# alipay/MMLRec-A-Unified-Multi-Task-and-Multi-Scenario-Learning-Benchmark-for-Recommendation

Hardware: AMD Instinct MI355X
Metric: train-step samples/sec, MMoE AliExpress-shape batch (higher is better)
Workload: dtype f32 (GEMMs: fp32-equivalent emulation on the 16-bit MFMA pipe with f32 accumulate -- two scaled fp16 planes per operand where the operand magnitudes travel with the tensors (batches >= 32 768), else three bf16 planes; max-norm error vs float64 3.3e-7 / 4.7e-7, fp32 MFMA 4.3e-7); 1 GPU; mmoe_ae30: 30 sparse fields, 12.49M rows (1e+07-row top table), E=8, mmoe 4 experts, experts [256, 128], gates [64], towers [64], adam lr 0.005; batch_per_gpu=65536, global_batch=65536, index_dist=zipf, table_update=dense_exact, dense_update_schedule=one launch after the scatter, gradients read for marked rows only, hip_graph=True, scatter_mode=deterministic, streams=1, early_fork=0, tables=single GPU

## Files before the change

### include/mmlrec.h

```cpp
#ifndef MMLREC_H
#define MMLREC_H

#include <stdint.h>

#ifdef __cplusplus
extern "C" {
#endif

#define MML_OK 0
#define MML_ERR_ARG (-1)
#define MML_ERR_HIP (-2)
#define MML_ERR_UNSUPPORTED (-3)

#define MML_MAX_FIELDS 64
#define MML_MAX_GROUP 16
#define MML_MAX_SRC 8
#define MML_MAX_EXPERTS 16
#define MML_MAX_GATES 8
#define MML_MAX_HEADS 8
#define MML_MAX_OPT_TENSORS 32
#define MML_AMAX_WORDS 8
#define MML_MAX_AMAX 64

typedef void* mml_stream_t;
// ... 525 lines not shown
  float* dV[2];
  float* dK[2];
  float* dQ[2];
  int64_t lddv[2], lddk[2], lddq[2];
  int64_t B;
  int32_t H;
  float sqrt_h;
} mml_attn2_desc;
int mml_attn2_fwd(const mml_attn2_desc* d, mml_stream_t stream);
int mml_attn2_bwd(const mml_attn2_desc* d, mml_stream_t stream);
int mml_esmm_combine(const float* p_raw, int64_t ldr, const float* y, int64_t ldy, const float* d_out, int64_t lddo,
                     float* p_out, int64_t ldo, float* d_raw, int64_t lddr, float* loss, int64_t B, mml_stream_t stream);
int mml_apg_features_fwd(const float* o1, int64_t ldo1, const float* s, int64_t lds, float* z, int64_t ldz, int64_t B,
                         int32_t k, int32_t E, int32_t Kf, mml_stream_t stream);
int mml_apg_features_bwd(const float* dz, int64_t lddz, const float* s, int64_t lds, float* do1, int64_t lddo1,
                         int64_t B, int32_t k, int32_t E, int32_t accumulate, mml_stream_t stream);
int mml_apg_weights(float* Wkk, float* bkk, float* Wb, float* Wcat, int64_t ldw, int32_t k, int32_t E, int32_t dir,
                    int32_t acc_kk, int32_t acc_bkk, int32_t acc_wb, mml_stream_t stream);
int mml_escm_combine(const float* p_raw, int64_t ldr, const float* y, int64_t ldy, const float* d_out, int64_t lddo,
                     float* p_out, int64_t ldo, float* d_raw, int64_t lddr, float* loss, int64_t B, float cf_w,
                     float global_w, mml_stream_t stream);
int mml_auc_segments(const float* pred, int64_t ldp, const float* y, int64_t ldy, int64_t n, int32_t cols, int32_t seg,
                     double* auc, mml_stream_t stream);
int32_t mml_auc_sorted_tile(void);
int64_t mml_auc_sorted_workspace_bytes(int64_t n, int32_t cols, int64_t seg);
int mml_auc_sorted(const float* pred, int64_t ldp, const float* y, int64_t ldy, const float* mask, int64_t ldm,
                   int32_t mask_cols, int64_t n, int32_t cols, int64_t seg, void* workspace, int64_t workspace_bytes,
                   double* auc, int64_t* counts, int32_t* status, mml_stream_t stream);
int mml_act_bwd(const float* y, const float* dy, float* dst, int64_t n, int32_t act, mml_stream_t stream);

typedef struct {
  float* param; const float* grad;
  float* state1;
  float* state2;
  int64_t n;
  float l1, l2;
  const uint32_t* skip_rows;
  int32_t row_elems;
  int32_t zero_grads;
  uint8_t* grad_marks;
  int64_t* acc64;
  const uint32_t* acc_amax;
  int32_t acc_shift;
  int32_t acc_pad_;
  uint8_t* warm_rows;
} mml_opt_tensor;
typedef struct {
  int32_t kind;
  int32_t step;
  const int32_t* step_dev;
  float lr, beta1, beta2, eps, alpha;
  int32_t zero_grad;
  int32_t max_blocks;
} mml_opt_hyper;
int mml_opt_step_dense(const mml_opt_tensor* tensors, int32_t n, const mml_opt_hyper* hyper, mml_stream_t stream);
int mml_opt_step_rows(float* const* tables, float* const* grad_tables, float* const* state1, float* const* state2,
                      uint32_t* const* seen, const int64_t* rowbase, int32_t F, int32_t E,
                      const int32_t* touched, const int32_t* touched_count, int32_t touched_cap,
                      int32_t* const* last ,
                      const mml_opt_hyper* hyper, mml_stream_t stream);
int mml_opt_catchup_rows(float* const* tables, float* const* state1, float* const* state2, int32_t* const* last,
                         const int64_t* rowbase, int32_t F, int32_t E, const int32_t* touched,
                         const int32_t* touched_count, int32_t touched_cap, const mml_opt_hyper* hyper,
                         mml_stream_t stream);
int mml_opt_catchup_dense(float* table, float* state1, float* state2, int32_t* last, int64_t V, int32_t E,
                          const mml_opt_hyper* hyper, mml_stream_t stream);
int mml_counter_update(int32_t* counter, int32_t delta, int32_t reset, mml_stream_t stream);

#ifdef __cplusplus
}
#endif
#endif
```

### mmlrec-a-unified-multi-task-and-multi-scenario-learning-benchmark-for-recommendation_amd/_lib.py

```python
import ctypes as C
import os

import torch

from . import build as _build

MAX_FIELDS, MAX_GROUP, MAX_SRC, MAX_EXPERTS, MAX_GATES, MAX_HEADS, MAX_OPT_TENSORS = 64, 16, 8, 16, 8, 8, 32
OPT_STREAM_MIN_PARAMS, OPT_HUGE_MIN_PARAMS, OPT_STREAM_MAX_TENSORS = 1 << 24, 1 << 22, 4
MAX_POOLED, POOL_MAX_LEN = 16, 256
POOL_COMBINERS = {"sum": 0, "mean": 1, "max": 2}
ACT_NONE, ACT_RELU, ACT_SIGMOID, ACT_SIGMOID2 = 0, 1, 2, 3
HEAD_OUT_SIGMOID, HEAD_OUT_IDENTITY = 0, 1
HEAD_LOSS_BCE, HEAD_LOSS_MSE, HEAD_LOSS_MAE = 0, 1, 2


def head_kind(out=HEAD_OUT_SIGMOID, loss=HEAD_LOSS_BCE):
    return (int(loss) << 8) | int(out)


ERR_ARG = -1
SCATTER_DET_CLEAR_MARKS, SCATTER_DET_AMAX_SUPPLIED, SCATTER_DET_DEFER_TOTALS = 1, 2, 4
OPT_SGD, OPT_ADAM, OPT_ADAGRAD, OPT_RMSPROP = 0, 1, 2, 3
OPT_KINDS = {"sgd": OPT_SGD, "adam": OPT_ADAM, "adagrad": OPT_ADAGRAD, "rmsprop": OPT_RMSPROP}

# ... 105 lines not shown
                ("amax_dH", fp), ("amax_dA", fp), ("K", i32), ("N", i32), ("n_hbias2", i32), ("mask_col", i32),
                ("head", i32), ("kind", i32)]


class TowerHeadGroup(C.Structure):
    _fields_ = [("n", i32), ("pad_", i32), ("M", i64), ("prob", fp), ("ldprob", i64), ("y", fp), ("ldy", i64),
                ("mask", fp), ("ldmask", i64), ("loss", fp), ("t", TowerHeadDesc * MAX_HEADS)]


class OptTensor(C.Structure):
    _fields_ = [("param", fp), ("grad", fp), ("state1", fp), ("state2", fp), ("n", i64), ("l1", C.c_float),
                ("l2", C.c_float), ("skip_rows", fp), ("row_elems", i32), ("zero_grads", i32), ("grad_marks", fp),
                ("acc64", fp), ("acc_amax", fp), ("acc_shift", i32), ("acc_pad_", i32), ("warm_rows", fp)]


class Copy2dDesc(C.Structure):
    _fields_ = [("src", fp), ("lds", i64), ("dst", fp), ("ldd", i64), ("rows", i64), ("cols", i32),
                ("accumulate", i32), ("amax_out", fp)]


class PreluDesc(C.Structure):
    _fields_ = [("z", fp), ("ldz", i64), ("y", fp), ("ldy", i64), ("rows", i64), ("cols", i32), ("pad_", i32),
                ("alpha", fp), ("amax_out", fp)]


class PreluBwdDesc(C.Structure):
    _fields_ = [("dy", fp), ("lddy", i64), ("z", fp), ("ldz", i64), ("dz", fp), ("lddz", i64), ("rows", i64),
                ("cols", i32), ("pad_", i32), ("alpha", fp), ("dalpha", fp), ("accumulate_dz", i32),
                ("accumulate_dalpha", i32), ("amax_out", fp)]


PCGRAD_MAX_TASKS = 8


class PcgradSeg(C.Structure):
    _fields_ = [("bank", fp * PCGRAD_MAX_TASKS), ("out", fp), ("rows", i64), ("ld", i64), ("cols", i32), ("pad_", i32),
                ("row_marks", fp)]


class SumProdDesc(C.Structure):
    _fields_ = [("out", fp), ("x", fp * 8), ("y", fp * 8), ("n", i64), ("n_terms", i32), ("accumulate", i32),
                ("deriv_of", fp), ("act", i32), ("pad_", i32), ("amax_out", fp)]


class Attn2Desc(C.Structure):
    _fields_ = [("V", fp * 2), ("K", fp * 2), ("Q", fp * 2), ("ldv", i64 * 2), ("ldk", i64 * 2), ("ldq", i64 * 2),
                ("out", fp), ("ldo", i64), ("A", fp), ("dout", fp), ("lddo", i64), ("dV", fp * 2), ("dK", fp * 2),
                ("dQ", fp * 2), ("lddv", i64 * 2), ("lddk", i64 * 2), ("lddq", i64 * 2), ("B", i64), ("H", i32),
                ("sqrt_h", C.c_float)]


class OptHyper(C.Structure):
    _fields_ = [("kind", i32), ("step", i32), ("step_dev", fp), ("lr", C.c_float), ("beta1", C.c_float),
                ("beta2", C.c_float), ("eps", C.c_float), ("alpha", C.c_float), ("zero_grad", i32), ("max_blocks", i32)]


_PP = C.POINTER
_SIGS = {
    "mml_version": (C.c_int, []),
    "mml_last_error": (C.c_char_p, []),
    "mml_device_caps": (C.c_int, [C.c_int, _PP(i64)]),
    "mml_stream_create_cu_range": (C.c_int, [C.c_int, C.c_int, C.c_int, _PP(C.c_void_p)]),
    "mml_stream_destroy": (C.c_int, [C.c_void_p]),
    "mml_gather_fwd": (C.c_int, [_PP(fp), _PP(i64), _PP(i32), i32, i32, fp, i64, i32, i32, i64, fp, i64, fp, fp]),
    "mml_gather_wgmax_len": (i64, [i32, i32, i32, i64]),
    "mml_gather_fwd_wgmax": (C.c_int, [_PP(fp), _PP(i64), _PP(i32), i32, i32, fp, i64, i32, i32, i64, fp, i64, fp, i64, fp, fp]),
    "mml_gather_fwd_mark": (C.c_int, [_PP(fp), _PP(i64), _PP(i32), i32, i32, fp, i64, i32, i32, i64, fp, i64, fp, fp, fp]),
    "mml_rows_compact": (C.c_int, [_PP(fp), _PP(i64), _PP(i64), i32, fp, fp, i32, fp, fp]),
    "mml_gather_fwd_idx32": (C.c_int, [_PP(fp), _PP(i64), i32, i32, fp, i64, fp, i64, i32, i64, fp, i64, fp, fp]),
    "mml_scatter_bwd": (C.c_int, [_PP(fp), _PP(i64), _PP(i32), i32, i32, fp, i64, i64, fp, i64, _PP(fp), _PP(i64),
                                  fp, fp, i32, fp, fp, fp]),
    "mml_scatter_bwd_det": (C.c_int, [_PP(fp), _PP(i64), _PP(i32), i32, i32, fp, i64, i64, fp, i64, _PP(fp), fp, fp, i32,
                                      fp, fp]),
    "mml_scatter_det_shift": (i32, [i64]),
    "mml_scatter_bwd_idx32": (C.c_int, [_PP(fp), _PP(i64), i32, i32, fp, i64, i64, fp, i64, _PP(fp), _PP(i64),
                                        fp, fp, i32, fp, fp, fp]),
    "mml_index_unique_idx32": (C.c_int, [_PP(i64), i32, i32, fp, i64, i64, _PP(fp), _PP(i64), fp, fp, i32, fp, fp, fp]),
    "mml_route_count": (C.c_int, [fp, i64, fp, i64, _PP(i32), _PP(i64), i32, i64, i32, fp, fp, fp]),
    "mml_route_place": (C.c_int, [fp, i64, fp, i64, _PP(i32), _PP(i64), _PP(i64), i32, i64, i32, fp, fp, fp, fp, fp]),
    "mml_rows_permute": (C.c_int, [fp, i64, fp, i32, i32, i64, fp, fp]),
    "mml_route_list_count": (C.c_int, [fp, fp, i32, _PP(i64), _PP(i64), i32, i32, fp, fp]),
    "mml_route_list_place": (C.c_int, [fp, fp, i32, _PP(i64), _PP(i64), _PP(i64), i32, i32, fp, fp, fp, fp]),
    "mml_lookup_slots": (C.c_int, [fp, i64, _PP(i32), _PP(i64), _PP(i64), i32, i64, fp, fp, fp, fp]),
    "mml_rows_clear": (C.c_int, [fp, fp, i32, _PP(i64), _PP(fp), i32, fp]),
    "mml_shard_rows": (C.c_int, [fp, i64, fp, i64, i32, i32, i32, i32, fp]),
    "mml_amax_batch": (C.c_int, [_PP(AmaxDesc), i32, fp]),
    "mml_amax_reset": (C.c_int, [fp, i64, fp]),
    "mml_gemm_planes_cut": (C.c_int, [C.POINTER(PlanesDesc), i32, fp]),
    "mml_gemm_set_mode": (C.c_int, [i32]),
    "mml_gemm_get_mode": (C.c_int, []),
    "mml_gemm_set_panel": (C.c_int, [i32]),
    "mml_gemm_set_ws": (C.c_int, [i32]),
    "mml_gemm_set_nt": (C.c_int, [i32]),
    "mml_gemm_nt_serves": (C.c_int, [_PP(GemmWgradDesc)]),
    "mml_gemm_os_serves": (C.c_int, [_PP(GemmDgradDesc), i32]),
    "mml_tower_head_serves": (C.c_int, [_PP(TowerHeadGroup)]),
    "mml_tower_head_workspace_bytes": (i64, [_PP(TowerHeadGroup)]),
    "mml_tower_head_fwd_bwd": (C.c_int, [_PP(TowerHeadGroup), fp, i64, i32, fp]),
    "mml_gemm_last_kernel": (C.c_char_p, []),
    "mml_gather_last_kernel": (C.c_char_p, []),
    "mml_gemm_set_wgrad_lds_pad": (C.c_int, [i32]),
    "mml_cast16_batch": (C.c_int, [_PP(Cast16Desc), i32, fp]),
    "mml_gather16_fwd": (C.c_int, [_PP(fp), _PP(i64), _PP(i32), i32, i32, fp, i64, i32, i32, i64, fp, i64, fp, fp]),
    "mml_g16_tn": (C.c_int, [_PP(G16TnDesc), i32, fp]),
    "mml_g16_wgrad_workspace_bytes": (i64, [_PP(G16WgradDesc), i32]),
    "mml_g16_wgrad": (C.c_int, [_PP(G16WgradDesc), i32, fp, i64, i32, fp]),
    "mml_g16_last_kernel": (C.c_char_p, []),
# ... 122 lines not shown
```

### mmlrec-a-unified-multi-task-and-multi-scenario-learning-benchmark-for-recommendation_amd/csrc/optim_ew.hip

```cpp
#include "common.hpp"
#include "fold_fixed.hpp"

#include <stdlib.h>

#ifndef MML_OPT_COLD_CB
#define MML_OPT_COLD_CB 8
#endif

namespace mml {

struct OptLaunch {
  mml_opt_tensor t[MML_MAX_OPT_TENSORS];
  int32_t n;
  int32_t variant;
  mml_opt_hyper h;
  int64_t chunk0[MML_MAX_OPT_TENSORS + 1];
  int32_t blk0[MML_MAX_OPT_TENSORS + 1];
  int32_t prop;
};
static_assert(sizeof(OptLaunch) <= 4096, "OptLaunch travels by value: the kernel-argument block holds 4 KB");

struct StepConsts {
  float step_size;
  float inv_bc2s;
// ... 117 lines not shown
      if (t0.x | t0.y) A64[2 * c] = lzero;
      if (t1.x | t1.y) A64[2 * c + 1] = lzero;
    };
    int64_t i = tid;
    if (PATH == OPT_UNROLL2 && !skip && !gm) {
      for (; i + stride < n4; i += 2 * stride) {
        const int64_t j = i + stride;
        f4 p0 = ld(P + i), p1 = ld(P + j);
        const f4 g0 = ld(G + i), g1 = ld(G + j);
        f4 a0 = S1 ? ld(S1 + i) : zero, a1 = S1 ? ld(S1 + j) : zero;
        f4 b0 = S2 ? ld(S2 + i) : zero, b1 = S2 ? ld(S2 + j) : zero;
        one(p0, g0, a0, b0);
        one(p1, g1, a1, b1);
        st(P + i, p0);
        st(P + j, p1);
        if (S1) { st(S1 + i, a0); st(S1 + j, a1); }
        if (S2) { st(S2 + i, b0); st(S2 + j, b1); }
        if (h.zero_grad && (g0.x != 0.f || g0.y != 0.f || g0.z != 0.f || g0.w != 0.f)) G[i] = zero;
        if (h.zero_grad && (g1.x != 0.f || g1.y != 0.f || g1.z != 0.f || g1.w != 0.f)) G[j] = zero;
      }
    }
    if (PATH == OPT_SKIP_U && skip) {
      for (; i + (U - 1) * stride < n4; i += U * stride) {
        f4 p[U], a[U], b[U];
        uint32_t w[U];
#pragma unroll
        for (int k = 0; k < U; ++k) {
          const int64_t row = row_of(i + k * stride);
          w[k] = (skip[row >> 5] >> (row & 31)) & 1u;
        }
#pragma unroll
        for (int k = 0; k < U; ++k) {
          const int64_t j = i + k * stride;
          if (!w[k]) {
            p[k] = ld(P + j);
            a[k] = S1 ? ld(S1 + j) : zero;
            b[k] = S2 ? ld(S2 + j) : zero;
          }
        }
#pragma unroll
        for (int k = 0; k < U; ++k) {
          if (w[k]) continue;
          const int64_t j = i + k * stride;
          const f4 g = zg ? zero : ld(G + j);
          one(p[k], g, a[k], b[k]);
          st(P + j, p[k]);
          if (S1) st(S1 + j, a[k]);
          if (S2) st(S2 + j, b[k]);
          if (h.zero_grad && (g.x != 0.f || g.y != 0.f || g.z != 0.f || g.w != 0.f)) G[j] = zero;
        }
      }
    }
    uint8_t* const wr = gm ? T.warm_rows : nullptr;
    if ((PATH == OPT_MARK_U || PATH == OPT_MARK_ACC_U) && wr && !skip) {
      constexpr int CB = MML_OPT_COLD_CB;
      for (; i < n4; i += CB * stride) {
        uint32_t lm = 0, wm = 0;
#pragma unroll
        for (int k = 0; k < CB; ++k) {
          const int64_t j = i + k * stride;
          const bool in = j < n4;
          const int64_t row = row_of(in ? j : i);
          const uint8_t mk = gm[row], wk = wr[row];
          lm |= (uint32_t)(in && mk != 0) << k;
          wm |= (uint32_t)(in && wk != 0) << k;
        }
        const uint32_t act = lm | wm;
        if (__builtin_amdgcn_ballot_w64(act != 0) == 0) continue;
#pragma unroll 1
        for (int kk = 0; kk < CB; kk += 2) {
          if (__builtin_amdgcn_ballot_w64(((act >> kk) & 3u) != 0) == 0) continue;
          f4 p[2], a[2], b[2], g[2];
          l2 t0[2], t1[2];
#pragma unroll
          for (int k = 0; k < 2; ++k) {
            const int64_t j = i + (kk + k) * stride;
            const bool on = (act >> (kk + k)) & 1u, lv = (lm >> (kk + k)) & 1u;
            p[k] = a[k] = b[k] = g[k] = zero;
            t0[k] = t1[k] = lzero;
            if (on) {
              p[k] = ld(P + j);
              if (S1) a[k] = ld(S1 + j);
              if (S2) b[k] = ld(S2 + j);
            }
            if (lv) {
              if (!zg) g[k] = ld(G + j);
              if (PATH == OPT_MARK_ACC_U && A64) {
                t0[k] = A64[2 * j];
                t1[k] = A64[2 * j + 1];
              }
            }
          }
#pragma unroll
          for (int k = 0; k < 2; ++k) {
            const int64_t j = i + (kk + k) * stride;
            const bool on = (act >> (kk + k)) & 1u, lv = (lm >> (kk + k)) & 1u;
            if (!on) continue;
            f4 gs = g[k];
            if (PATH == OPT_MARK_ACC_U && A64 && lv) add_totals(gs, t0[k], t1[k], j);
            one(p[k], gs, a[k], b[k]);
            st(P + j, p[k]);
            if (S1) st(S1 + j, a[k]);
            if (S2) st(S2 + j, b[k]);
            if (h.zero_grad && (g[k].x != 0.f || g[k].y != 0.f || g[k].z != 0.f || g[k].w != 0.f)) G[j] = zero;
            const int64_t row = row_of(j);
            if (lv && (j << 2) == row * re) {
              gm[row] = 0;
// ... 618 lines not shown
}

extern "C" int mml_opt_step_dense(const mml_opt_tensor* tensors, int32_t n, const mml_opt_hyper* hyper,
                                  mml_stream_t stream) {
  int rc = check_hyper(hyper, "mml_opt_step_dense");
  if (rc) return rc;
  MML_REQUIRE(n >= 0 && (n == 0 || tensors), "mml_opt_step_dense: bad tensor array");
  int i = 0;
  while (i < n) {
    OptLaunch L{};
    L.h = *hyper;
    int64_t total = 0, chunks = 0;
    while (i < n && L.n < MML_MAX_OPT_TENSORS) {
      const mml_opt_tensor& t = tensors[i];
      MML_REQUIRE(t.param && t.grad && t.n >= 0, "mml_opt_step_dense: tensor %d malformed", i);
      MML_REQUIRE(hyper->kind == MML_OPT_SGD || t.state1, "mml_opt_step_dense: tensor %d needs state1", i);
      MML_REQUIRE(hyper->kind != MML_OPT_ADAM || t.state2, "mml_opt_step_dense: tensor %d needs state2 (Adam)", i);
      MML_REQUIRE(!t.skip_rows || (t.row_elems > 0 && t.row_elems % 4 == 0 && t.n % t.row_elems == 0 &&
                                   aligned16(t.param)),
                  "mml_opt_step_dense: tensor %d: skip_rows needs row_elems %% 4 == 0 dividing n and a 16-byte aligned "
                  "parameter (16-byte chunks must lie inside one row)", i);
      if (t.acc64) {
        MML_REQUIRE(t.grad_marks && !t.skip_rows && t.acc_amax && aligned16(t.acc64) && t.acc_shift >= 4 &&
                        t.acc_shift <= 28,
                    "mml_opt_step_dense: tensor %d: acc64 (deferred totals of mml_scatter_bwd_det) needs grad_marks, no "
                    "skip_rows, a 16-byte aligned int64 array, acc_amax and acc_shift = mml_scatter_det_shift(B)", i);
      }
      if (t.grad_marks) {
        const int cpr = t.row_elems / 4;
        MML_REQUIRE(t.row_elems > 0 && t.row_elems % 4 == 0 && cpr <= 64 && (cpr & (cpr - 1)) == 0 &&
                        t.n % t.row_elems == 0 && !t.skip_rows && aligned16(t.param) && aligned16(t.grad) &&
                        (!t.state1 || aligned16(t.state1)) && (!t.state2 || aligned16(t.state2)),
                    "mml_opt_step_dense: tensor %d: grad_marks needs 16-byte aligned [rows, row_elems] tensors with "
                    "row_elems / 4 a power of two <= 64 and no skip_rows", i);
      }
      if (t.warm_rows) {
        MML_REQUIRE(t.grad_marks && t.l1 == 0.f && t.l2 == 0.f,
                    "mml_opt_step_dense: tensor %d: warm_rows needs grad_marks and no regulariser (a regulariser moves a "
                    "row whose moments and gradient are zero)", i);
      }
      L.chunk0[L.n] = chunks;
      L.t[L.n++] = t;
      total += t.n;
      chunks += cdiv(t.n, 4);
      ++i;
    }
    L.chunk0[L.n] = chunks;
    if (total == 0) continue;
    static int variant = -1;
    if (variant < 0) {
      const char* e = getenv("MMLREC_OPT_VARIANT");
      variant = e ? atoi(e) : 0;
    }
    L.variant = variant | (hyper->max_blocks > 0 ? 4 : 0);
    int64_t nmax = 0;
    for (int k = 0; k < L.n; ++k) nmax = L.t[k].n > nmax ? L.t[k].n : nmax;
    bool all_gm = true, all_skip = true, none = true, any_acc = false;
    for (int k = 0; k < L.n; ++k) {
      any_acc = any_acc || L.t[k].acc64;
      all_gm = all_gm && L.t[k].grad_marks && !L.t[k].skip_rows;
      all_skip = all_skip && L.t[k].skip_rows;
      none = none && !L.t[k].grad_marks && !L.t[k].skip_rows;
    }
    const bool many = L.n > 4 && all_gm;
    MML_REQUIRE(!any_acc || all_gm, "mml_opt_step_dense: a launch with acc64 tensors takes grad_marks on every tensor");
    if (total >= ((int64_t)1 << 24) && (L.n <= 4 || many)) {
      int64_t bx = cdiv(cdiv(nmax, 4), 256);
      if (bx > 256 * 8) bx = 256 * 8;
      if (hyper->max_blocks > 0 && bx * L.n > hyper->max_blocks) bx = cdiv(hyper->max_blocks, L.n);
      dim3 grid((unsigned)bx, (unsigned)L.n);
      bool all_warm = true;
      for (int k = 0; k < L.n; ++k) all_warm = all_warm && L.t[k].warm_rows;
      static int cold_wgs = -1;
      if (cold_wgs < 0) {
        const char* e = getenv("MMLREC_OPT_COLD_WGS");
        cold_wgs = e ? atoi(e) : 256 * 8;
        if (cold_wgs < 1 || cold_wgs > 256 * 8) cold_wgs = 256 * 8;
      }
      const int64_t wg_cap = all_warm ? cold_wgs : 256 * 8;
      if (many) {
        int64_t want = 0;
        for (int k = 0; k < L.n; ++k) {
          const int64_t need = cdiv(cdiv(L.t[k].n, 4), 256);
          want += need > wg_cap ? wg_cap : (need < 1 ? 1 : need);
        }
        const bool capped = hyper->max_blocks > 0 && want > hyper->max_blocks;
        int64_t tb = capped ? hyper->max_blocks : want;
        if (tb < L.n) tb = L.n;
        int64_t at = 0;
        for (int k = 0; k < L.n; ++k) {
          L.blk0[k] = (int32_t)at;
          const int64_t need = cdiv(cdiv(L.t[k].n, 4), 256);
          int64_t nb = capped ? tb * L.t[k].n / total : (need > wg_cap ? wg_cap : need);
          if (nb > need) nb = need;
          if (nb < 1) nb = 1;
          at += nb;
        }
        L.blk0[L.n] = (int32_t)at;
        L.prop = 1;
        grid = dim3((unsigned)at, 1);
      }
      static int u_mark = -1;
      if (u_mark < 0) {
        const char* e = getenv("MMLREC_OPT_U");
        u_mark = e ? atoi(e) : 2;
      }
      hipStream_t st = to_stream(stream);
// ... 250 lines not shown
```

### mmlrec-a-unified-multi-task-and-multi-scenario-learning-benchmark-for-recommendation_amd/ops.py

```python
import ctypes as C

import os

import torch

from . import _lib as L

_workspaces = {}


def _stream():
    return torch.cuda.current_stream().cuda_stream


_masked_streams = {}


def cu_range_stream(device, cu_lo, cu_hi):
    idx = device.index if device.index is not None else torch.cuda.current_device()
    key = (idx, int(cu_lo), int(cu_hi))
    st = _masked_streams.get(key)
    if st is None:
        h = C.c_void_p()
        L.check(L.load().mml_stream_create_cu_range(idx, int(cu_lo), int(cu_hi), C.byref(h)))
# ... 779 lines not shown
                    (b.shape[-1] > 1 and b.stride(-1) != 1)):
                raise L.MMLError("pcgrad: banks and out of a segment must be float32 views of one shape and pitch")
        rows, cols = (1, ref.shape[0]) if ref.dim() == 1 else ref.shape
        for k, b in enumerate(banks):
            d.bank[k] = b.data_ptr() if b is not None else None
        d.out = L.ptr(sg.get("out"))
        d.rows, d.cols, d.ld = rows, cols, (cols if ref.dim() == 1 else _ld(ref))
        marks = sg.get("marks")
        if marks is not None and (marks.dtype != torch.uint8 or marks.numel() < rows or not marks.is_contiguous()):
            raise L.MMLError("pcgrad: marks must be a contiguous uint8 tensor with one byte per row")
        d.row_marks = L.ptr(marks)
        if need_out and sg.get("out") is None:
            raise L.MMLError("pcgrad combine: a segment without `out`")
    return arr


def pcgrad_gram(segs, T, gram=None):
    arr = make_pcgrad_segs(segs, T)
    dev = next(b for b in segs[0]["banks"] if b is not None).device
    if gram is None:
        gram = torch.empty((T, T), dtype=torch.float64, device=dev)
    nbytes = int(L.load().mml_pcgrad_workspace_bytes(arr, len(segs), T))
    ws = workspace(nbytes, dev)
    L.check(L.load().mml_pcgrad_gram(arr, len(segs), T, gram.data_ptr(), ws.data_ptr(), nbytes, _stream()),
            "mml_pcgrad_gram")
    return gram


def pcgrad_weights(gram, order, w=None, fired=None):
    _need_gpu(gram, order)
    T = gram.shape[0]
    if gram.dtype != torch.float64 or order.dtype != torch.int32 or order.numel() != T * T or gram.numel() != T * T \
            or not gram.is_contiguous() or not order.is_contiguous():
        raise L.MMLError("pcgrad_weights: gram [T, T] float64 and order [T, T] int32, contiguous")
    if w is None:
        w = torch.empty(2 * T, dtype=torch.float32, device=gram.device)
    if fired is None:
        fired = torch.empty((T, T), dtype=torch.int32, device=gram.device)
    L.check(L.load().mml_pcgrad_weights(gram.data_ptr(), order.data_ptr(), T, w.data_ptr(), fired.data_ptr(), _stream()),
            "mml_pcgrad_weights")
    return w, fired


def pcgrad_combine(segs, T, w):
    _need_gpu(w)
    arr = make_pcgrad_segs(segs, T, need_out=True)
    L.check(L.load().mml_pcgrad_combine(arr, len(segs), T, w.data_ptr(), _stream()), "mml_pcgrad_combine")


def act_bwd(y, dy, dst, act):
    L.check(L.load().mml_act_bwd(y.data_ptr(), dy.data_ptr(), dst.data_ptr(), y.numel(), act, _stream()), "mml_act_bwd")


def make_hyper(kind, lr, step=1, step_dev=None, zero_grad=False, max_blocks=0):
    h = L.OptHyper()
    h.kind = L.OPT_KINDS[kind] if isinstance(kind, str) else int(kind)
    h.step = int(step)
    h.step_dev = L.ptr(step_dev)
    h.lr = float(lr)
    h.beta1, h.beta2 = 0.9, 0.999
    h.eps = {L.OPT_ADAM: 1e-8, L.OPT_ADAGRAD: 1e-10, L.OPT_RMSPROP: 1e-8}.get(h.kind, 0.0)
    h.alpha = 0.99
    h.zero_grad = int(zero_grad)
    h.max_blocks = int(max_blocks)
    return h


def make_opt_tensors(entries):
    arr = (L.OptTensor * len(entries))()
    for d, ent in zip(arr, entries):
        p, g, s1, s2 = ent[:4]
        d.param, d.grad, d.state1, d.state2, d.n = p.data_ptr(), g.data_ptr(), L.ptr(s1), L.ptr(s2), p.numel()
        d.l1, d.l2 = ent[4] if len(ent) > 4 and ent[4] else (0.0, 0.0)
        if len(ent) > 5 and ent[5] is not None:
            d.skip_rows, d.row_elems, d.zero_grads = ent[5].data_ptr(), p.shape[1], 1
        if len(ent) > 6 and ent[6] is not None:
            d.grad_marks, d.row_elems = ent[6].data_ptr(), p.shape[1]
        if len(ent) > 7 and ent[7] is not None:
            d.acc64, d.acc_amax, d.acc_shift = ent[7][0].data_ptr(), ent[7][1].data_ptr(), int(ent[7][2])
        if len(ent) > 8 and ent[8] is not None:
            d.warm_rows = ent[8].data_ptr()
    return arr


def opt_step_dense(entries, hyper):
    arr = make_opt_tensors(entries)
    L.check(L.load().mml_opt_step_dense(arr, len(entries), C.byref(hyper), _stream()), "mml_opt_step_dense")


def opt_step_rows(tables, grad_tables, state1, state2, seen, rowbase, touched, touched_count, hyper, last=None):
    F, E = len(tables), tables[0].shape[1]
    rb = (L.i64 * (F + 1))(*rowbase)
    L.check(L.load().mml_opt_step_rows(_ptr_array(tables), _ptr_array(grad_tables),
                                       _ptr_array(state1) if state1 is not None else None,
                                       _ptr_array(state2) if state2 is not None else None,
                                       _ptr_array(seen), rb, F, E, touched.data_ptr(), touched_count.data_ptr(),
                                       touched.numel(), _ptr_array(last) if last is not None else None,
                                       C.byref(hyper), _stream()), "mml_opt_step_rows")


def index_unique(vocab, cols, E, X, seen, rowbase, touched, touched_count, status=None, marks=None):
    F = len(vocab)
    L.check(L.load().mml_index_unique((L.i64 * F)(*vocab), (L.i32 * F)(*cols), F, E, X.data_ptr(), _ld(X), X.shape[0],
                                      _ptr_array(seen), (L.i64 * (F + 1))(*rowbase), touched.data_ptr(),
                                      touched_count.data_ptr(), touched.numel(), L.ptr(marks), L.ptr(status), _stream()),
            "mml_index_unique")


# ... 188 lines not shown
```

### mmlrec-a-unified-multi-task-and-multi-scenario-learning-benchmark-for-recommendation_amd/optimizer.py

```python
import ctypes as C
import dataclasses
import os
import typing

import torch

from . import _lib as L
from . import engine as E
from . import ops


@dataclasses.dataclass(frozen=True)
class OptKnobs:
    lazy_min_params: int = 1 << 22
    auto_table_update: str = "lazy_exact"
    early_blocks: int = 0
    tail_blocks: int = 1 << 20
    opt_u: typing.Optional[int] = None
    one_launch: bool = False
    variant: int = 0
    scatter_old: bool = False
    cold_rows: bool = True

    @classmethod
    def from_env(cls, env=None):
        env = os.environ if env is None else env
        u = env.get("MMLREC_OPT_U")
        return cls(lazy_min_params=int(env.get("MMLREC_LAZY_MIN_PARAMS", str(1 << 22))),
                   auto_table_update=env.get("MMLREC_AUTO_TABLE_UPDATE", "lazy_exact"),
                   early_blocks=int(env.get("MMLREC_EARLY_BLOCKS", "0")),
                   tail_blocks=int(env.get("MMLREC_TAIL_BLOCKS", str(1 << 20))),
                   opt_u=int(u) if u is not None else None,
                   one_launch=env.get("MMLREC_OPT_ONE_LAUNCH", "0") == "1",
                   variant=int(env.get("MMLREC_OPT_VARIANT", "0")),
                   scatter_old=bool(env.get("MMLREC_SCATTER_OLD")),
                   cold_rows=env.get("MMLREC_OPT_COLD_ROWS", "1") != "0")


TABLE_UPDATES = ("dense_exact", "sparse_rows", "lazy_exact")
BYTES_PER_PARAM = {"sgd": 12, "adam": 28, "adagrad": 20, "rmsprop": 20}


def resolve_table_update(kind, requested, widths, one_table_per_field, table_params, table_reg, knobs):
    mode = requested
    if requested == "auto":
        if kind in ("sgd", "adagrad"):
            mode = "sparse_rows"
        else:
            ok = (len(widths) == 1 and widths <= {4, 8, 16} and one_table_per_field and
                  table_params > knobs.lazy_min_params and knobs.auto_table_update == "lazy_exact")
            mode = "lazy_exact" if ok else "dense_exact"
        if table_reg:
            mode = "dense_exact"
    if mode == "lazy_exact" and kind in ("sgd", "adagrad"):
        mode = "sparse_rows"
    if mode not in TABLE_UPDATES:
        raise ValueError("table_update must be auto, dense_exact, sparse_rows or lazy_exact")
    return mode


def opt_dense_symbol(numel, ntensors, form=0, opt_u=None):
    if not L.opt_dense_streams(numel, ntensors, form in (3, 4)):
        return "opt_flat_kernel"
    u = {0: 1, 1: 1, 2: 4, 3: 2 if opt_u is None else opt_u, 4: 4 if opt_u == 4 else 2}[form]
    return "opt_dense_kernel<true, %d, %d>" % (form, u)


class DenseLaunch(typing.NamedTuple):
    tables: tuple
    marked: bool
    form: int
    bytes: float
    kernel: str


def dense_table_launches(kind, numels, rows, marks, split_dense, cap, det_deferred, knobs, det_exact=True):
    n = len(numels)
    big = [i for i in range(n) if numels[i] >= L.OPT_HUGE_MIN_PARAMS]
    if len(big) > L.OPT_STREAM_MAX_TENSORS or sum(numels[i] for i in big) < L.OPT_STREAM_MIN_PARAMS:
        big = []
    small = [i for i in range(n) if i not in big]
    one_launch = bool(big and small and cap > 0 and n <= L.MAX_OPT_TENSORS and not split_dense and all(marks) and
                      knobs.one_launch)
    if det_deferred:
        if not (det_exact and L.opt_takes_det_totals(numels, all(marks), split_dense)):
            raise L.MMLError("the deterministic scatter deferred its totals to a marked dense update of exactly its "
                             "tables")
        one_launch = True
    if one_launch:
        big, small = small + big, []
    per = BYTES_PER_PARAM[kind] - (4 if split_dense else 0)
    out = []
    for grp in (big, small):
        if not grp:
            continue
        marked = grp is big and all(marks[i] for i in grp)
        numel = sum(numels[i] for i in grp)
        nbytes = float(per) * numel
        form = (4 if det_deferred else 3 if (cap > 0 and marked) else 2 if (cap > 0 and split_dense) else
                1 if (knobs.variant & 2 and not marked and not split_dense) else 0)
        if marked:
            nbytes += sum(rows[i] - 4.0 * numels[i] for i in grp)
        out.append(DenseLaunch(tuple(grp), marked, form, nbytes, opt_dense_symbol(numel, len(grp), form, knobs.opt_u)))
    return out


WARM_KINDS = ("adam", "rmsprop", "adagrad")


def launch_trusts_warm_map(kind, marked, table_reg, knobs, sharded=False):
    return bool(marked and kind in WARM_KINDS and not table_reg and knobs.cold_rows and not sharded)


class TableRows:

    def __init__(self, vocab, device, cap):
        self.rowbase = [0]
        for v in vocab:
            self.rowbase.append(self.rowbase[-1] + int(v))
        self.seen = [torch.zeros((int(v) + 31) // 32, dtype=torch.int32, device=device) for v in vocab]
        self.marks = torch.zeros(ops.marks_bytes(vocab), dtype=torch.uint8, device=device)
        self.touched = torch.zeros(max(int(cap), 1), dtype=torch.int32, device=device)
        self.count = torch.zeros(1, dtype=torch.int32, device=device)


class ParamStore:

    def __init__(self, model, device):
        self.device = device
        self.model = model
        tables, dense = [], []
        for name, p in model.named_parameters():
            (tables if name.startswith("embedding_dict.") else dense).append((name, p))
        self.sig = tuple(p.data_ptr() for _, p in tables + dense)
        total = sum(p.numel() for _, p in dense)
        self.arena = torch.zeros(max(total, 1), dtype=torch.float32, device=device)
        self.pvals = {}
        off = 0
        for name, p in dense:
            g = self.arena[off:off + p.numel()].view(p.shape)
            off += p.numel()
            self.pvals[name] = E.PVal(p.data, g, name)
            self.pvals[name].stable = True
        self.table_names = [n for n, _ in tables]
        for name, p in tables:
            self.pvals[name] = E.PVal(p.data, None, name, is_table=True)
        par = getattr(model, "_parallel", None)
        if par is not None and par.mode == "row_sharded":
            self.pvals["embedding_shard"] = E.PVal(par.shard, None, "embedding_shard", is_table=True)
            self.table_names = ["embedding_shard"]
        self.table_grads_ready = False
        self.opt = None
        self.rows = None
        self.rows_names = None
        self._grad_marks_key = self._det_key = None
        self.extra = {}

    def ensure_table_grads(self):
        if not self.table_grads_ready:
            for n in self.table_names:
                pv = self.pvals[n]
                pv.grad = torch.zeros_like(pv.data)
                pv.needs_grad = True
            self.table_grads_ready = True

    def ensure_rows(self, cap, names=None):
# ... 107 lines not shown
        return c["pre"] + c["early"] + c["mlp"] + c["tables"]

    def split_dense_ok(self, widths):
        return (self.table_update == "dense_exact" and not self.table_reg() and
                all(w <= 16 and w % 4 == 0 for w in widths))

    def can_split_dense(self, plan):
        gop = plan.ops[0] if plan.ops else None
        if not isinstance(gop, E.GatherOp) or isinstance(gop, E.PooledGatherOp):
            return False
        return self.split_dense_ok([t.data.shape[1] for t in gop.tables])

    def calls_split(self, plan, split_dense=False):
        knobs = OptKnobs.from_env()
        pre = [(L.load().mml_counter_update, (self.step_dev.data_ptr(), 1, 0))]
        if self.table_update == "lazy_exact":
            pre += self._lazy_pre_calls(plan)
        split_dense = bool(split_dense) and self.can_split_dense(plan)
        if split_dense and getattr(plan.ops[0], "mark_rows", None) is None:
            pre += self.index_pre_calls(plan)
        reg = self._reg_map()
        treg = self.table_reg(reg)
        names = [n for n in self.store.table_names if self.store.pvals[n].written]
        if treg and self.table_update != "dense_exact":
            raise NotImplementedError("l2_reg_embedding / l1 on the tables makes every row's gradient non-zero: use "
                                      "table_update='dense_exact' (the reference's own dense optimizer)")
        hyper = ops.make_hyper(self.kind, self.lr, step=0, step_dev=self.step_dev, zero_grad=False)
        plan.keep.append(hyper)
        mlp = self._mlp_calls(plan, reg, hyper)
        early, tables = [], []
        if names and self.table_update == "dense_exact":
            (early if split_dense else tables).extend(self._dense_table_calls(plan, names, treg, split_dense, knobs))
        if names and (self.table_update != "dense_exact" or split_dense):
            tables += self._row_update_calls(plan, names, hyper, knobs)
        return {"pre": pre, "early": early, "mlp": mlp, "tables": tables}

    def _mlp_calls(self, plan, reg, hyper):
        dense = [(pv, n) for n, pv in self.store.pvals.items()
                 if not pv.is_table and pv.grad is not None and (pv.written or pv.data.data_ptr() in reg)]
        if not dense:
            return []
        arr = ops.make_opt_tensors([(pv.data, pv.grad) + self.state[n] + (reg.get(pv.data.data_ptr()),)
                                    for pv, n in dense])
        plan.keep.append(arr)
        numel = sum(pv.data.numel() for pv, _ in dense)
        return [(L.load().mml_opt_step_dense, (arr, len(dense), C.byref(hyper)),
                 dict(kernel=opt_dense_symbol(numel, len(dense)), bytes=float(BYTES_PER_PARAM[self.kind]) * numel))]

    def _dense_table_calls(self, plan, names, treg, split_dense, knobs):
        st = self.store
        tabs = [st.pvals[n] for n in names]
        cap = knobs.early_blocks if split_dense else knobs.tail_blocks
        hz = ops.make_hyper(self.kind, self.lr, step=0, step_dev=self.step_dev, zero_grad=not split_dense,
                            max_blocks=cap)
        plan.keep.append(hz)
        seen_of = dict(zip(st.rows_names, st.rows.seen)) if split_dense else {}
        gop = plan.ops[0] if plan.ops else None
        marks_of = {} if split_dense else st.grad_marks_by_table(gop)
        dd = getattr(gop, "det_deferred", None)
        launches = dense_table_launches(
            self.kind, [t.data.numel() for t in tabs], [t.data.shape[0] for t in tabs],
            [id(t) in marks_of for t in tabs], split_dense, cap, dd is not None, knobs,
            det_exact=dd is None or {id(t) for t in tabs} == {id(t) for t in gop.tables})
        acc_of = {id(t): a for t, a in zip(gop.tables, gop.deterministic["acc64"])} if dd else {}
        calls = []
        for ln in launches:
            trust = launch_trusts_warm_map(self.kind, ln.marked, treg, knobs, sharded=not isinstance(gop, E.GatherOp))
            if not trust:
                self.all_rows_warm([names[i] for i in ln.tables])
            arr = ops.make_opt_tensors([(tabs[i].data, tabs[i].grad) + self.state[names[i]] +
                                        (treg, seen_of.get(names[i]), marks_of[id(tabs[i])] if ln.marked else None,
                                         (acc_of[id(tabs[i])], dd["slot"], dd["shift"]) if dd else None,
                                         self.warm_map(names[i]) if trust else None)
                                        for i in ln.tables])
            plan.keep.append(arr)
            m = dict(kernel=ln.kernel, bytes=ln.bytes)
            if dd:
                m.update(det_acc64=True, ptrs=[dd["slot"].data_ptr()] + [a.data_ptr() for a in acc_of.values()])
            calls.append((L.load().mml_opt_step_dense, (arr, len(ln.tables), C.byref(hz)), m))
        return calls

    def _row_update_calls(self, plan, names, hyper, knobs):
        rows = self.store.rows
        a = self._row_arrays(plan, names, grads=True, last=self.table_update == "lazy_exact")
        self.all_rows_warm(names)
        calls = [(L.load().mml_opt_step_rows, (a["param"], a["grad"], a["s1"], a["s2"], a["seen"], a["rowbase"], a["F"],
                                               a["E"], rows.touched.data_ptr(), rows.count.data_ptr(),
                                               rows.touched.numel(), a["last"], C.byref(hyper)),
                  dict(kernel="opt_rows_kernel"))]
        if a["E"] not in (4, 8, 16) or knobs.scatter_old:
            calls.append((L.load().mml_counter_update, (rows.count.data_ptr(), 0, 1)))
        return calls

    def _row_arrays(self, plan, names, grads=False, state=True, last=False):
        st, rows = self.store, self.store.rows
        tabs = [st.pvals[n] for n in names]
        F = len(tabs)
        a = dict(F=F, E=tabs[0].data.shape[1], vocab=(L.i64 * F)(*[t.data.shape[0] for t in tabs]),
                 param=ops._ptr_array([t.data for t in tabs]), seen=ops._ptr_array(rows.seen),
                 rowbase=(L.i64 * (F + 1))(*rows.rowbase),
                 grad=ops._ptr_array([t.grad for t in tabs]) if grads else None,
                 s1=ops._ptr_array([self.state[n][0] for n in names]) if state and self.kind != "sgd" else None,
                 s2=ops._ptr_array([self.state[n][1] for n in names]) if state and self.kind == "adam" else None,
                 last=ops._ptr_array([self.last[n] for n in names]) if last else None)
        plan.keep += [v for v in a.values() if isinstance(v, C.Array)]
        return a

# ... 82 lines not shown
```

Before: 58.87 million samples/s.

## Compact live rows per wave in dense Adam table update cold-row loop

Replaces the per-element cold-row loop in the marked dense table optimizer with a per-wave scan that reads four mark and warm bytes per lane. Live rows are compacted into a shared-memory list using ballot prefix sums, or handled directly when a span is dense. The optimizer update then runs only over live row elements, cutting the idle lanes and scattered byte reads of the old CB loop over the large tables. The cost is more complex control flow, shared-memory use, and a dependence on 4-byte alignment of the mark arrays, with the old loop kept behind a fallback flag.

Result: faster. 60.53 million samples/s (median of 6 runs) (+2.8%).

```diff
diff --git a/include/mmlrec.h b/include/mmlrec.h
--- a/include/mmlrec.h
+++ b/include/mmlrec.h
@@ -601,6 +601,7 @@
   float lr, beta1, beta2, eps, alpha;
   int32_t zero_grad;
   int32_t max_blocks;
+  int32_t cold_loop;
 } mml_opt_hyper;
 int mml_opt_step_dense(const mml_opt_tensor* tensors, int32_t n, const mml_opt_hyper* hyper, mml_stream_t stream);
 int mml_opt_step_rows(float* const* tables, float* const* grad_tables, float* const* state1, float* const* state2,
diff --git a/mmlrec-a-unified-multi-task-and-multi-scenario-learning-benchmark-for-recommendation_amd/_lib.py b/mmlrec-a-unified-multi-task-and-multi-scenario-learning-benchmark-for-recommendation_amd/_lib.py
--- a/mmlrec-a-unified-multi-task-and-multi-scenario-learning-benchmark-for-recommendation_amd/_lib.py
+++ b/mmlrec-a-unified-multi-task-and-multi-scenario-learning-benchmark-for-recommendation_amd/_lib.py
@@ -181,7 +181,8 @@
 
 class OptHyper(C.Structure):
     _fields_ = [("kind", i32), ("step", i32), ("step_dev", fp), ("lr", C.c_float), ("beta1", C.c_float),
-                ("beta2", C.c_float), ("eps", C.c_float), ("alpha", C.c_float), ("zero_grad", i32), ("max_blocks", i32)]
+                ("beta2", C.c_float), ("eps", C.c_float), ("alpha", C.c_float), ("zero_grad", i32), ("max_blocks", i32),
+                ("cold_loop", i32)]
 
 
 _PP = C.POINTER
diff --git a/mmlrec-a-unified-multi-task-and-multi-scenario-learning-benchmark-for-recommendation_amd/csrc/optim_ew.hip b/mmlrec-a-unified-multi-task-and-multi-scenario-learning-benchmark-for-recommendation_amd/csrc/optim_ew.hip
--- a/mmlrec-a-unified-multi-task-and-multi-scenario-learning-benchmark-for-recommendation_amd/csrc/optim_ew.hip
+++ b/mmlrec-a-unified-multi-task-and-multi-scenario-learning-benchmark-for-recommendation_amd/csrc/optim_ew.hip
@@ -193,7 +193,139 @@
       }
     }
     uint8_t* const wr = gm ? T.warm_rows : nullptr;
-    if ((PATH == OPT_MARK_U || PATH == OPT_MARK_ACC_U) && wr && !skip) {
+    const bool compact = !(L.variant & 8) && wr &&
+                         ((reinterpret_cast<uintptr_t>(gm) | reinterpret_cast<uintptr_t>(wr)) & 3) == 0;
+    if ((PATH == OPT_MARK_U || PATH == OPT_MARK_ACC_U) && compact && !skip) {
+      constexpr int RPL = 4, SPAN = 64 * RPL;
+      constexpr int DENSE_PCT = 15;
+      constexpr int WAVES = 4;
+      __shared__ uint16_t live_rows[WAVES][SPAN];
+      const int lane = threadIdx.x & 63;
+      const int wv = __builtin_amdgcn_readfirstlane((int)(threadIdx.x >> 6));
+      uint16_t* const lst = live_rows[wv];
+      const int csh = rsh - 2;
+      const int64_t rows = T.n >> rsh;
+      const int64_t nspan = (rows + SPAN - 1) / SPAN, nwv = (int64_t)nblk * WAVES;
+      auto nz80 = [](uint32_t x) { return (x | ((x & 0x7f7f7f7fu) + 0x7f7f7f7fu)) & 0x80808080u; };
+      auto pack4 = [](uint32_t t) { return ((t >> 7) & 1u) | ((t >> 14) & 2u) | ((t >> 21) & 4u) | ((t >> 28) & 8u); };
+      auto scan = [&](int64_t s, uint32_t& mk, uint32_t& wk) {
+        const int64_t r0 = s * SPAN + lane * RPL;
+        mk = wk = 0u;
+        if (r0 + RPL <= rows) {
+          mk = *reinterpret_cast<const uint32_t*>(gm + r0);
+          wk = *reinterpret_cast<const uint32_t*>(wr + r0);
+        } else {
+#pragma unroll
+          for (int k = 0; k < RPL; ++k)
+            if (r0 + k < rows) {
+              mk |= (uint32_t)gm[r0 + k] << (8 * k);
+              wk |= (uint32_t)wr[r0 + k] << (8 * k);
+            }
+        }
+      };
+      int64_t s = (int64_t)lblk * WAVES + wv;
+      uint32_t mk = 0, wk = 0;
+      if (s < nspan) scan(s, mk, wk);
+      for (; s < nspan; s += nwv) {
+        uint32_t mkn = 0, wkn = 0;
+        if (s + nwv < nspan) scan(s + nwv, mkn, wkn);
+        const uint32_t lm = pack4(nz80(mk)), wm = pack4(nz80(wk));
+        const uint32_t act = lm | wm;
+        if (__builtin_amdgcn_ballot_w64(act != 0) != 0) {
+          const int64_t row0 = s * SPAN;
+          const uint32_t cnt = (uint32_t)__builtin_popcount(act);
+          uint32_t pre = 0;
+          int nlive = 0;
+#pragma unroll
+          for (int bit = 0; (1 << bit) <= RPL; ++bit) {
+            const uint64_t bal = __builtin_amdgcn_ballot_w64(((cnt >> bit) & 1u) != 0);
+            pre += __builtin_amdgcn_mbcnt_hi((uint32_t)(bal >> 32), __builtin_amdgcn_mbcnt_lo((uint32_t)bal, 0u)) << bit;
+            nlive += __builtin_popcountll(bal) << bit;
+          }
+          const bool dense = nlive * 100 >= SPAN * DENSE_PCT;
+          if (!dense) {
+            __builtin_amdgcn_fence(__ATOMIC_RELEASE, "wavefront");
+            __builtin_amdgcn_wave_barrier();
+#pragma unroll
+            for (int k = 0; k < RPL; ++k)
+              if ((act >> k) & 1u)
+                lst[pre++] = (uint16_t)((lane * RPL + k) | (((lm >> k) & 1u) << 14) | (((wm >> k) & 1u) << 15));
+            __builtin_amdgcn_fence(__ATOMIC_RELEASE, "wavefront");
+            __builtin_amdgcn_wave_barrier();
+          }
+          if (lm) {
+            const int64_t r0 = row0 + lane * RPL;
+            if (r0 + RPL <= rows) {
+              *reinterpret_cast<uint32_t*>(gm + r0) = 0u;
+              const uint32_t set = (nz80(mk) & ~nz80(wk)) >> 7;
+              if (set) *reinterpret_cast<uint32_t*>(wr + r0) = wk | set;
+            } else {
+#pragma unroll
+              for (int k = 0; k < RPL; ++k)
+                if ((lm >> k) & 1u) {
+                  gm[r0 + k] = 0;
+                  if (!((wm >> k) & 1u)) wr[r0 + k] = 1;
+                }
+            }
+          }
+          const int items = (dense ? SPAN : nlive) << csh;
+#pragma unroll 1
+          for (int b0 = 0; b0 < items; b0 += 128) {
+            f4 p[2], a[2], b[2], g[2];
+            l2 t0[2], t1[2];
+            int64_t jj[2];
+            bool on[2], lv[2];
+#pragma unroll
+            for (int k = 0; k < 2; ++k) {
+              const int it = b0 + 64 * k + lane;
+              const int ent = it >> csh;
+              on[k] = it < items;
+              uint32_t e;
+              if (dense) {
+                const uint32_t src = (uint32_t)__shfl((int)(lm | (act << 16)), (ent / RPL) & 63);
+                on[k] = on[k] && ((src >> (16 + (ent & (RPL - 1)))) & 1u);
+                e = (uint32_t)ent | (((src >> (ent & (RPL - 1))) & 1u) << 14);
+              } else {
+                e = on[k] ? lst[ent] : 0u;
+              }
+              lv[k] = on[k] && ((e >> 14) & 1u);
+              const int64_t j = ((row0 + (int64_t)(e & 0x3fffu)) << csh) | (int64_t)(it & ((1 << csh) - 1));
+              jj[k] = j;
+              p[k] = a[k] = b[k] = g[k] = zero;
+              t0[k] = t1[k] = lzero;
+              if (on[k]) {
+                p[k] = ld(P + j);
+                if (S1) a[k] = ld(S1 + j);
+                if (S2) b[k] = ld(S2 + j);
+              }
+              if (lv[k]) {
+                if (!zg) g[k] = ld(G + j);
+                if (PATH == OPT_MARK_ACC_U && A64) {
+                  t0[k] = A64[2 * j];
+                  t1[k] = A64[2 * j + 1];
+                }
+              }
+            }
+#pragma unroll
+            for (int k = 0; k < 2; ++k) {
+              if (!on[k]) continue;
+              const int64_t j = jj[k];
+              f4 gs = g[k];
+              if (PATH == OPT_MARK_ACC_U && A64 && lv[k]) add_totals(gs, t0[k], t1[k], j);
+              one(p[k], gs, a[k], b[k]);
+              st(P + j, p[k]);
+              if (S1) st(S1 + j, a[k]);
+              if (S2) st(S2 + j, b[k]);
+              if (h.zero_grad && (g[k].x != 0.f || g[k].y != 0.f || g[k].z != 0.f || g[k].w != 0.f)) G[j] = zero;
+            }
+          }
+        }
+        mk = mkn;
+        wk = wkn;
+      }
+      i = n4;
+    }
+    if ((PATH == OPT_MARK_U || PATH == OPT_MARK_ACC_U) && wr && !skip && !compact) {
       constexpr int CB = MML_OPT_COLD_CB;
       for (; i < n4; i += CB * stride) {
         uint32_t lm = 0, wm = 0;
@@ -918,7 +1050,7 @@
       const char* e = getenv("MMLREC_OPT_VARIANT");
       variant = e ? atoi(e) : 0;
     }
-    L.variant = variant | (hyper->max_blocks > 0 ? 4 : 0);
+    L.variant = variant | (hyper->max_blocks > 0 ? 4 : 0) | (hyper->cold_loop == 1 ? 8 : 0);
     int64_t nmax = 0;
     for (int k = 0; k < L.n; ++k) nmax = L.t[k].n > nmax ? L.t[k].n : nmax;
     bool all_gm = true, all_skip = true, none = true, any_acc = false;
diff --git a/mmlrec-a-unified-multi-task-and-multi-scenario-learning-benchmark-for-recommendation_amd/ops.py b/mmlrec-a-unified-multi-task-and-multi-scenario-learning-benchmark-for-recommendation_amd/ops.py
--- a/mmlrec-a-unified-multi-task-and-multi-scenario-learning-benchmark-for-recommendation_amd/ops.py
+++ b/mmlrec-a-unified-multi-task-and-multi-scenario-learning-benchmark-for-recommendation_amd/ops.py
@@ -855,8 +855,9 @@
     L.check(L.load().mml_act_bwd(y.data_ptr(), dy.data_ptr(), dst.data_ptr(), y.numel(), act, _stream()), "mml_act_bwd")
 
 
-def make_hyper(kind, lr, step=1, step_dev=None, zero_grad=False, max_blocks=0):
+def make_hyper(kind, lr, step=1, step_dev=None, zero_grad=False, max_blocks=0, cold_loop=0):
     h = L.OptHyper()
+    h.cold_loop = int(cold_loop)
     h.kind = L.OPT_KINDS[kind] if isinstance(kind, str) else int(kind)
     h.step = int(step)
     h.step_dev = L.ptr(step_dev)
diff --git a/mmlrec-a-unified-multi-task-and-multi-scenario-learning-benchmark-for-recommendation_amd/optimizer.py b/mmlrec-a-unified-multi-task-and-multi-scenario-learning-benchmark-for-recommendation_amd/optimizer.py
--- a/mmlrec-a-unified-multi-task-and-multi-scenario-learning-benchmark-for-recommendation_amd/optimizer.py
+++ b/mmlrec-a-unified-multi-task-and-multi-scenario-learning-benchmark-for-recommendation_amd/optimizer.py
@@ -21,6 +21,7 @@
     variant: int = 0
     scatter_old: bool = False
     cold_rows: bool = True
+    cold_compact: bool = True
 
     @classmethod
     def from_env(cls, env=None):
@@ -34,7 +35,8 @@
                    one_launch=env.get("MMLREC_OPT_ONE_LAUNCH", "0") == "1",
                    variant=int(env.get("MMLREC_OPT_VARIANT", "0")),
                    scatter_old=bool(env.get("MMLREC_SCATTER_OLD")),
-                   cold_rows=env.get("MMLREC_OPT_COLD_ROWS", "1") != "0")
+                   cold_rows=env.get("MMLREC_OPT_COLD_ROWS", "1") != "0",
+                   cold_compact=env.get("MMLREC_OPT_COLD_COMPACT", "1") != "0")
 
 
 TABLE_UPDATES = ("dense_exact", "sparse_rows", "lazy_exact")
@@ -112,6 +114,10 @@
     return bool(marked and kind in WARM_KINDS and not table_reg and knobs.cold_rows and not sharded)
 
 
+def cold_loop_of(knobs):
+    return 0 if knobs.cold_compact else 1
+
+
 class TableRows:
 
     def __init__(self, vocab, device, cap):
@@ -325,7 +331,7 @@
         tabs = [st.pvals[n] for n in names]
         cap = knobs.early_blocks if split_dense else knobs.tail_blocks
         hz = ops.make_hyper(self.kind, self.lr, step=0, step_dev=self.step_dev, zero_grad=not split_dense,
-                            max_blocks=cap)
+                            max_blocks=cap, cold_loop=cold_loop_of(knobs))
         plan.keep.append(hz)
         seen_of = dict(zip(st.rows_names, st.rows.seen)) if split_dense else {}
         gop = plan.ops[0] if plan.ops else None
```
